# leducthanhig/image-restoration-models

Measured on AMD Instinct MI355X. Metric: images/sec + PSNR, Restormer motion-deblur 1280x720, higher is better.
Workload: dtype f32 (1x1 convs: fp32 emulated by 3 fp16 MFMAs on hi/lo operand splits with fp32 accumulation, error vs float64 at the level of an fp32 chain; everything else exact f32; value_exact_f32: f32 MFMA everywhere); 1 GPU; Restormer motion-deblur (WithBias LN, 26.13M params, synthetic weights seed 42) on 1280x720x3 uint8 GoPro-shaped synthetic frames; 6 tiles 512x512 (overlap 96) per frame; a step = 4 frame(s) per GPU, their 24 tiles in one batched forward; global_batch=4, tile=512, overlap=96, parallelism=per-image shard x1, no data-path collective

## Files before the change

### image-restoration-models_amd/_hip.py

```python
from __future__ import annotations

import ctypes as C
import os

import torch

_HERE = os.path.dirname(os.path.abspath(__file__))
LIB_PATH = os.path.join(_HERE, "libirm_hip.so")

ACT_NONE, ACT_RELU, ACT_GELU, ACT_SILU, ACT_RELU6 = 0, 1, 2, 3, 4
LN_NONE, LN_WITHBIAS, LN_BIASFREE = 0, 1, 2

_P, _L, _I, _F, _D = C.c_void_p, C.c_long, C.c_int, C.c_float, C.c_double

SIGNATURES = {
    "irm_version": [],
    "irm_ln_stats_f32": [_P, _L, _P, _I, _I, _I, _F, _P],
    "irm_gemm1x1_f32": [_P, _L, _P, _L, _P, _L, _P, _L, _P, _P, _P, _P, _I, _I, _I, _I, _I, _I, _I, _I, _P, _F, _P, _P],
    "irm_gemm1x1_f16x3_f32": [_P, _L, _P, _L, _P, _L, _P, _L, _P, _P, _P, _P, _I, _I, _I, _I, _I, _I, _I, _I, _P, _F, _P, _P],
    "irm_ln_split_f16": [_P, _L, _P, _P, _I, _F, _F, _P, _I, _I, _I, _P],
    "irm_ln_gemm_presplit_f16x3_f32": [_P, _P, _L, _P, _P, _I, _F, _F, _P, _L, _P, _F, _I, _I, _I, _I, _I, _P],
    "irm_ln_gemm_presplit_cl_f16x3_f32": [_P, _P, _L, _P, _P, _I, _F, _F, _P, _L, _P, _F, _I, _I, _I, _I, _I, _I, _P],
    "irm_gdfn_tail_f16x3_f32": [_P, _L, _P, _P, _P, _P, _L, _F, _I, _I, _I, _I, _I, _I, _P],
    "irm_gemm_presplit_f16x3_f32": [_P, _P, _P, _L, _P, _F, _I, _I, _I, _I, _I, _I, _I, _I, _P],
# ... 30 lines not shown
    "irm_selective_scan_f32": [_P, _P, _P, _P, _P, _P, _P, _P, _P, _P, _P, _I, _I, _I, _I, _I, _I, _P],
    "irm_losh_combine_f32": [_P, _P, _P, _P, _P, _P, _P, _P, _L, _P, _L, _I, _I, _I, _I, _F, _P],
    "irm_window_blend": [_P, _P, _P, _P, _I, _P, _P, _I, _I, _I, _I, _I, _I, _I, _I, _I, _I, _F, _F, _P],
    "irm_window_blend_scaled": [_P, _P, _P, _P, _I, _P, _P, _I, _I, _I, _I, _I, _I, _I, _I, _I, _I, _I, _F, _F, _P],
    "irm_frame_metrics": [_P, _P, _I, _I, _I, _I, _I, _D, _P, _P, _P, _L, _P],
    "irm_imresize_bicubic": [_P, _I, _P, _I, _P, _P, _P, _P, _I, _I, _I, _I, _I, _I, _P],
    "irm_frame_metrics_basicsr": [_P, _P, _I, _I, _I, _I, _I, _I, _I, _I, _P, _P, _P, _L, _P],
    "irm_niqe_features": [_P, _I, _I, _I, _I, _I, _I, _I, _P, _P, _P, _L, _P],
    "irm_dihedral_chop_f32": [_P, _P, _P, _L, _I, _I, _I, _I, _I, _I, _I, _P],
    "irm_ensemble_merge_f32": [_P, _P, _P, _L, _I, _I, _I, _I, _I, _I, _P],
}

SIGNATURES_HALF = {
    "irm_conv3x3_h_in_f32": [_P, _P, _L, _P, _L, _P, _I, _I, _I, _I, _I, _I, _P],
    "irm_conv3x3_h_f16": [_P, _F, _P, _L, _P, _L, _P, _L, _P, _I, _I, _I, _I, _I, _I, _I, _I, _P],
    "irm_conv3x3_h_out_f32": [_P, _P, _L, _P, _L, _P, _L, _P, _I, _I, _I, _I, _I, _I, _P],
}

SIGNATURES_FRAMES = {
    "irm_frame_minmax_f32": [_P, _L, _P, _P, _L, _P],
    "irm_tile_extract_f32": [_P, _P, _P, _P, _P, _I, _I, _I, _I, _I, _I, _I, _I, _I, _P],
    "irm_window_blend_f32": [_P, _P, _P, _P, _P, _I, _I, _I, _I, _I, _I, _I, _I, _I, _I, _I, _P],
}

SIGNATURES_GRAM = {
    "irm_dw_gram_cm_f16x3_f32": [_P, _L, _P, _P, _P, _P, _I, _I, _I, _I, _I, _P],
}

SIGNATURES_YUV = {
    "irm_yuv420_to_rgb_f32": [_P, _P, _P, _I, _L, _L, _I, _I, _I, _I, _I, _I, _I, _I, _P, _P],
    "irm_rgb_f32_to_yuv420": [_P, _P, _P, _P, _I, _L, _L, _I, _I, _I, _I, _I, _I, _I, _I, _P],
}

_lib = None


class HipLibraryError(RuntimeError):
    pass


def load():
    global _lib, LIB_PATH
    if _lib is None:
        if os.environ.get("IRM_HIP_LIB"):
            LIB_PATH = os.path.abspath(os.environ["IRM_HIP_LIB"])
        if not os.path.exists(LIB_PATH):
            raise HipLibraryError(
                f"{LIB_PATH} not found: build it with `python -c 'import __graft_entry__ as g; g.build()'` "
                "(make -C image-restoration-models_amd/csrc).  There is no CPU fallback.")
        lib = C.CDLL(LIB_PATH)
        for name, argtypes in {**SIGNATURES, **SIGNATURES_HALF, **SIGNATURES_FRAMES, **SIGNATURES_GRAM,
                               **SIGNATURES_YUV}.items():
            fn = getattr(lib, name)
            fn.argtypes = argtypes
            fn.restype = _I
        _lib = lib
    return _lib


def _stream() -> int:
    return torch.cuda.current_stream().cuda_stream


def ptr(t):
    if t is None:
        return None
    if isinstance(t, int):
        return t
    assert t.is_cuda, "HIP kernels need device tensors"
    return t.data_ptr()


def call(name: str, *args):
    rc = getattr(load(), name)(*args, _stream())
    if rc != 0:
        raise HipLibraryError(f"{name} failed with status {rc} "
                              f"({'invalid arguments' if rc == -1 else 'HIP launch error'})")



def pack_gemm_weight(w: torch.Tensor) -> torch.Tensor:
    w = w.detach().reshape(w.shape[0], -1).float()
    m, k = w.shape
    mt, ks = (m + 15) // 16, 4 * ((k + 15) // 16)
    wpad = torch.zeros(mt * 16, ks * 4, dtype=torch.float32, device=w.device)
# ... 402 lines not shown
```

### image-restoration-models_amd/csrc/conv3x3_f16.hip

```cpp
#include "conv_epilogue.h"


#define CF_TH 8
#define CF_TW IRM_CONV_TW
#define CF_PLANE 400
#define CF_HC 34
#define CF_NP 340
#define CF_PXB 160
#define CF_RAWB (7 * 512 * 16)
#define CF_IMGB (CF_NP * CF_PXB)
#define CF_NRAW 7


__device__ __forceinline__ float cf_res(float v, float r, int mode) {
    if (mode == 1) return v + r;
    if (mode == 2) return r - v;
    return fminf(fmaxf(tanhf(v) + r, -1.0f), 1.0f);
}

struct ConvF16Args {
    const float* Wp;
    const float* X; long x_bs;
    float* Y; long y_bs;
    const float* R; long r_bs;
    const float* bias;
    int Ci, Co, H, W, mtiles, S;
    int relu1, res_mode, relu2, store_mode, tiles_x;
    float inv_s;
    float slope;
    int ps_r;
};


template <int CT, int NCH = 1>
__global__ __launch_bounds__(512, 2) void conv3x3_f16x3_kernel(ConvF16Args a) {
    constexpr int TT = CT * NCH;
    constexpr int NG = 3 * NCH;
    constexpr int WGB = 3 * CT * 2048;
    constexpr int NW = (WGB / 16 + 511) / 512;
    extern __shared__ __attribute__((aligned(16))) float smem[];
    char* lds = reinterpret_cast<char*>(smem);
    char* raw = lds;
    char* img = lds + CF_RAWB;
    char* wbuf = img + CF_IMGB;

    const int tid = threadIdx.x, lane = tid & 63, wave = __builtin_amdgcn_readfirstlane(tid >> 6);
    const int g = lane >> 4, r = lane & 15;
    const int b = blockIdx.z;
    const int ty0 = (blockIdx.x / a.tiles_x) * CF_TH, tx0 = (blockIdx.x % a.tiles_x) * CF_TW;
    const float* X = a.X + (long)b * a.x_bs;
    const long plane = (long)a.H * a.W;
    const int S = a.S;
    const int nchunks = (a.mtiles + TT - 1) / TT;
    const int my_chunks = (nchunks - (int)blockIdx.y + (int)gridDim.y - 1) / (int)gridDim.y;

    long xoff[CF_NRAW];
    int xch[CF_NRAW];
    bool xok[CF_NRAW];
#pragma unroll
    for (int j = 0; j < CF_NRAW; ++j) {
        const int q = j * 512 + tid;
        const int ch = q / 100, rem = q - ch * 100, row = rem / 10, chunk = rem - row * 10;
        const int gy = ty0 - 1 + row, gx = tx0 - 4 + chunk * 4;
        xch[j] = ch;
        xok[j] = q < 3200 && gy >= 0 && gy < a.H && gx >= 0 && gx < a.W;
        xoff[j] = (long)ch * plane + (long)gy * a.W + gx;
    }
    const float* const zero_page = irm_zero_page;
    auto issue_raw = [&](int s) {
#pragma unroll
        for (int j = 0; j < CF_NRAW; ++j) {
            const bool ok = xok[j] && s * 32 + xch[j] < a.Ci;
            const float* src = ok ? X + (long)s * 32 * plane + xoff[j] : zero_page;
            __builtin_amdgcn_global_load_lds((const __attribute__((address_space(1))) void*)src,
                                             (__attribute__((address_space(3))) void*)(raw + (j * 512 + wave * 64) * 16), 16, 0, 0);
        }
    };
    auto issue_w = [&](int mt0, int n) {
        const int sc = n / 3, tg = n - 3 * sc, s = sc / NCH, chn = sc - s * NCH;
#pragma unroll
        for (int j = 0; j < NW; ++j) {
            const int cb = min(j * 512 + wave * 64, WGB / 16 - 64);
            const int q = cb + lane;
            const int ct = q / 384, rem = q - ct * 384;
            const int mt = min(mt0 + chn * CT + ct, a.mtiles - 1);
            const float* src = a.Wp + ((((long)mt * S + s) * 9 + tg * 3) * 2) * 256 + rem * 4;
            __builtin_amdgcn_global_load_lds((const __attribute__((address_space(1))) void*)src,
                                             (__attribute__((address_space(3))) void*)(wbuf + (n & 1) * WGB + cb * 16), 16, 0, 0);
        }
    };

    f32x4 acc[2][TT];
    float* Y = a.Y + (long)b * a.y_bs;
    const float* R = a.R ? a.R + (long)b * a.r_bs : nullptr;

    for (int ci = 0; ci < my_chunks; ++ci) {
        const int mt0 = ((int)blockIdx.y + ci * (int)gridDim.y) * TT;
#pragma unroll
        for (int p = 0; p < 2; ++p)
#pragma unroll
            for (int c = 0; c < TT; ++c) acc[p][c] = (f32x4){0.f, 0.f, 0.f, 0.f};
        __builtin_amdgcn_s_barrier();
        issue_raw(0);
        issue_w(mt0, 0);
        for (int s = 0; s < S; ++s) {
            irm_wait_vmcnt<0>();
            __builtin_amdgcn_s_barrier();
#pragma unroll
            for (int it = 0; it < 3; ++it) {
                const int item = it * 512 + tid;
                if (item < 4 * CF_NP) {
                    const int cg = item / CF_NP, px = item - cg * CF_NP;
                    const int row = px / CF_HC, col = px - row * CF_HC;
                    const float* rp = reinterpret_cast<const float*>(raw) + (8 * cg) * CF_PLANE + row * 40 + col + 3;
                    irm_h8 hi, lo;
                    float xs[8];
#pragma unroll
                    for (int e = 0; e < 8; ++e) xs[e] = irm_sat_h(__fmul_rn(rp[e * CF_PLANE], 0.0625f));
                    irm_split8(xs, hi, lo);
                    *reinterpret_cast<irm_h8*>(img + px * CF_PXB + cg * 16) = hi;
                    *reinterpret_cast<irm_h8*>(img + px * CF_PXB + 64 + cg * 16) = lo;
                }
            }
            asm volatile("s_waitcnt lgkmcnt(0)" ::: "memory");
            __builtin_amdgcn_s_barrier();
            issue_w(mt0, NG * s + 1);
            if (s + 1 < S) issue_raw(s + 1);
#pragma unroll
            for (int gi = 0; gi < NG; ++gi) {
                const int n = NG * s + gi, tg = gi % 3, chn = gi / 3;
                if (gi == 1) {
                    if (s + 1 < S) irm_wait_vmcnt<CF_NRAW>(); else irm_wait_vmcnt<0>();
                    __builtin_amdgcn_s_barrier();
                    issue_w(mt0, n + 1);
                } else if (gi > 1) {
                    irm_wait_vmcnt<0>();
                    __builtin_amdgcn_s_barrier();
                    if (gi + 1 < NG || s + 1 < S) issue_w(mt0, n + 1);
                }
                const char* wb = wbuf + (n & 1) * WGB;
#pragma unroll
                for (int tl = 0; tl < 3; ++tl) {
                    const int dy = tg, dx = tl;
                    irm_h8 ah[2], al[2];
#pragma unroll
                    for (int p = 0; p < 2; ++p) {
                        const int pi = (wave + dy) * CF_HC + 16 * p + r + dx;
                        ah[p] = *reinterpret_cast<const irm_h8*>(img + pi * CF_PXB + 16 * g);
                        al[p] = *reinterpret_cast<const irm_h8*>(img + pi * CF_PXB + 64 + 16 * g);
                    }
#pragma unroll
                    for (int c = 0; c < CT; ++c) {
                        const irm_h8 wh = *reinterpret_cast<const irm_h8*>(wb + ((c * 3 + tl) * 2) * 1024 + lane * 16);
                        const irm_h8 wl = *reinterpret_cast<const irm_h8*>(wb + ((c * 3 + tl) * 2 + 1) * 1024 + lane * 16);
#pragma unroll
                        for (int p = 0; p < 2; ++p) {
                            f32x4& t = acc[p][chn * CT + c];
                            t = irm_mfma3_f16(ah[p], al[p], wh, wl, t);
                        }
                    }
                }
            }
        }
#pragma unroll
        for (int c = 0; c < TT; ++c) {
            const int co = (mt0 + c) * 16 + r;
            const bool row_ok = mt0 + c < a.mtiles && co < a.Co;
            const float bv = (a.bias && row_ok) ? a.bias[co] : 0.0f;
#pragma unroll
            for (int p = 0; p < 2; ++p) {
                const int y = ty0 + wave, x = tx0 + p * 16 + g * 4;
                float v[4];
#pragma unroll
                for (int e = 0; e < 4; ++e) {
                    v[e] = fmaf(acc[p][c][e], a.inv_s, bv);
                    if (a.relu1 == 1) v[e] = fmaxf(v[e], 0.0f);
                    else if (a.relu1 == 2) v[e] = v[e] > 0.0f ? v[e] : v[e] * a.slope;
                }
                if (!row_ok || y >= a.H || x >= a.W) continue;
                if (a.store_mode == 0) {
                    const long off = (long)co * plane + (long)y * a.W + x;
                    if (a.res_mode) {
                        const float4 rr = *reinterpret_cast<const float4*>(R + off);
                        const float rv[4] = {rr.x, rr.y, rr.z, rr.w};
#pragma unroll
                        for (int e = 0; e < 4; ++e) v[e] = cf_res(v[e], rv[e], a.res_mode);
                    }
                    if (a.relu2) {
#pragma unroll
                        for (int e = 0; e < 4; ++e) v[e] = fmaxf(v[e], 0.0f);
                    }
                    *reinterpret_cast<float4*>(Y + off) = make_float4(v[0], v[1], v[2], v[3]);
                } else if (a.store_mode == 1) {
                    const int oh = a.H >> 1, ow = a.W >> 1;
                    const long op = (long)oh * ow;
                    const int oc = co * 4 + (y & 1) * 2;
                    const long o = (long)(y >> 1) * ow + (x >> 1);
                    *reinterpret_cast<float2*>(Y + (long)oc * op + o) = make_float2(v[0], v[2]);
                    *reinterpret_cast<float2*>(Y + (long)(oc + 1) * op + o) = make_float2(v[1], v[3]);
                } else if (a.ps_r == 2) {
                    const int ow = a.W * 2;
                    const long op = (long)a.H * 2 * ow;
                    const int oc = co >> 2, i = (co >> 1) & 1, jx = co & 1;
                    float* o = Y + (long)oc * op + (long)(2 * y + i) * ow + 2 * x + jx;
#pragma unroll
                    for (int e = 0; e < 4; ++e) o[2 * e] = v[e];
                } else {
                    const int pr = a.ps_r, ow = a.W * pr;
                    const long op = (long)a.H * pr * ow;
                    const int oc = co / (pr * pr), i = (co / pr) % pr, jx = co % pr;
                    float* o = Y + (long)oc * op + (long)(pr * y + i) * ow + pr * x + jx;
#pragma unroll
                    for (int e = 0; e < 4; ++e) o[pr * e] = v[e];
                }
            }
        }
    }
}

template <int CT, int NCH = 1>
static int launch_conv_f16(const ConvF16Args& a, int B, int ygroups, hipStream_t stream) {
    const size_t lds = (size_t)CF_RAWB + CF_IMGB + 2 * (3 * CT * 2048);
    static_assert((size_t)CF_RAWB + CF_IMGB + 2 * (3 * CT * 2048) <= 160 * 1024, "LDS");
    IRM_ALLOW_BIG_LDS((&conv3x3_f16x3_kernel<CT, NCH>));
    const int tiles_y = (a.H + CF_TH - 1) / CF_TH;
    dim3 grid(a.tiles_x * tiles_y, ygroups, B);
    hipLaunchKernelGGL((conv3x3_f16x3_kernel<CT, NCH>), grid, dim3(512), lds, stream, a);
    return irm_launch_status();
}

extern "C" int irm_conv3x3_f16x3_ep_f32(const float* wp_split, float inv_scale, const float* x, long x_bs, float* y,
                                        long y_bs, const float* res, long r_bs, const float* bias, int B, int Ci, int Co,
                                        int H, int W, int act1, float slope, int res_mode, int relu2, int store_mode,
                                        int shuffle, int ct, int ygroups, hipStream_t stream) {
    ConvF16Args a;
    if (int rc = irm_conv_common(a, wp_split, x, x_bs, y, y_bs, res, r_bs, bias, B, Ci, Co, H, W, act1, slope, res_mode,
                                 relu2, store_mode, shuffle, ct, ygroups)) return rc;
    if ((W & 3) || (x_bs & 3) || (y_bs & 3) || (r_bs & 3)) return IRM_EINVAL;
    if (!irm_aligned16(x) || !irm_aligned16(y) || !irm_aligned16(res) || !irm_aligned16(wp_split)) return IRM_EINVAL;
    a.S = (Ci + 31) / 32; a.inv_s = inv_scale;
    switch (ct) {
        case 1: return launch_conv_f16<1>(a, B, ygroups, stream);
        case 2: return launch_conv_f16<2>(a, B, ygroups, stream);
        case 3: return launch_conv_f16<3>(a, B, ygroups, stream);
        case 4: return launch_conv_f16<4>(a, B, ygroups, stream);
        case 8: return launch_conv_f16<4, 2>(a, B, ygroups, stream);
        case 12: return launch_conv_f16<4, 3>(a, B, ygroups, stream);
        default: return IRM_EINVAL;
    }
}

extern "C" int irm_conv3x3_f16x3_f32(const float* wp_split, float inv_scale, const float* x, long x_bs, float* y, long y_bs,
                                     const float* res, long r_bs, const float* bias, int B, int Ci, int Co, int H, int W,
                                     int relu1, int res_mode, int relu2, int store_mode, int ct, int ygroups,
                                     hipStream_t stream) {
    return irm_conv3x3_f16x3_ep_f32(wp_split, inv_scale, x, x_bs, y, y_bs, res, r_bs, bias, B, Ci, Co, H, W, relu1 ? 1 : 0,
                                    0.0f, res_mode, relu2, store_mode, 2, ct, ygroups, stream);
}
```

### image-restoration-models_amd/ops.py

```python
from __future__ import annotations

import os

import torch

from . import _hip
from ._hip import ACT_GELU, ACT_NONE, ACT_RELU, ACT_RELU6, ACT_SILU, LN_BIASFREE, LN_NONE, LN_WITHBIAS


class KernelTimer:

    def __init__(self, detail=False, only=None):
        self.records = []
        self.detail = detail
        self.only = None if only is None else frozenset(only)
        self._chain = {}
        self._done = {}
        self._since = 0

    def _fold(self, k, e0, e1, fl, by):
        d = self._done.setdefault(k, dict(launches=0, ms=0.0, flops=0.0, bytes=0.0))
        d["launches"] += 1
        d["ms"] += e0.elapsed_time(e1)
        d["flops"] += fl
# ... 400 lines not shown
        ygroups = max(1, min(nchunks, -(-target_blocks() // blocks)))
    return ct, ygroups


def conv3x3(wp, x, y, ci: int, co: int, *, bias=None, relu1=False, res=None, res_mode=0, relu2=False,
            store_mode=0, ct: int | None = None, ygroups: int | None = None, leaky: float | None = None, shuffle: int = 2):
    _chk(x, "x"), _chk(y, "y")
    B, _, H, W = x.shape
    nbytes = 4.0 * B * H * W * (ci + co + (co if res is not None else 0))
    if leaky is not None and relu1:
        raise ValueError("conv3x3: relu1 and leaky are exclusive")
    act1, slope = (2, float(leaky)) if leaky is not None else (int(bool(relu1)), 0.0)
    extra = (f" ps{shuffle}" if shuffle != 2 else "") + (f" leaky{slope:g}" if leaky is not None else "")
    if isinstance(wp, _hip.ConvWeight):
        aligned = (W % 4 == 0 and _bs(x) % 4 == 0 and _bs(y) % 4 == 0 and _bs(res) % 4 == 0 and x.data_ptr() % 16 == 0
                   and y.data_ptr() % 16 == 0 and (res is None or res.data_ptr() % 16 == 0))
        if wp.raw is not None and aligned and store_mode == 0 and act1 < 2:
            _launch("conv3x3_thin", 18.0 * B * ci * co * H * W, nbytes, "irm_conv3x3_thin_f32", _hip.ptr(wp.raw), _hip.ptr(x),
                    _bs(x), _hip.ptr(y), _bs(y), _hip.ptr(res), _bs(res), _hip.ptr(bias), B, ci, co, H, W, int(relu1),
                    int(res_mode), int(relu2), tag=f"ci{ci} co{co} {H}x{W} B{B}")
            return
        wp = (wp.split, wp.inv_scale) if (wp.split is not None and aligned) else wp.exact
    if isinstance(wp, tuple):
        kernel, entry, lead = "conv3x3_f16x3", "irm_conv3x3_f16x3_ep_f32", (_hip.ptr(wp[0]), float(wp[1]))
    else:
        kernel, entry, lead = "conv3x3", "irm_conv3x3_ep_f32", (_hip.ptr(wp),)
    ct, ygroups = plan_conv3x3(co, H, W, B, split=isinstance(wp, tuple), ct=ct, ygroups=ygroups)
    _launch(kernel, 18.0 * B * ci * co * H * W, nbytes, entry, *lead, _hip.ptr(x), _bs(x), _hip.ptr(y), _bs(y),
            _hip.ptr(res), _bs(res), _hip.ptr(bias), B, ci, co, H, W, act1, slope, int(res_mode), int(relu2),
            int(store_mode), int(shuffle), ct, ygroups,
            tag=f"ci{ci} co{co} {H}x{W} B{B} ct{ct} yg{ygroups} st{store_mode}{extra}")


def transpose(src: torch.Tensor, dst: torch.Tensor, R: int, C: int):
    B = src.shape[0]
    _launch("transpose", 0.0, 8.0 * B * R * C, "irm_transpose_f32", _hip.ptr(src), src.stride(0), _hip.ptr(dst),
            dst.stride(0), B, R, C, tag=f"R{R} C{C} B{B}")


def scan_is_flat(D: int, N: int, R: int) -> bool:
    return (N, R) in ((1, 4), (16, 4)) and D % 64 != 0


def scan_plan(B: int, L: int, D: int, flat: bool = False):
    DB = (D + 63) // 64
    waves = -(-4 * D // 64) if flat else 4 * DB
    nchunk = max(1, min(-(-L // 32), -(-3072 // (B * waves))))
    chunk = max(32, -(-(-(-L // nchunk)) // 8) * 8)
    return chunk, -(-L // chunk), DB


def selective_scan(xT, pT, ids, dtw, dtb, A, Dskip, yT, state, sdt, ysum, B, L, D, N, R, chunk):
    flops = B * 4.0 * L * D * (2 * R + 9 * N + 12)
    nbytes = 4.0 * B * L * (D + 4 * (R + 2 * N) + 4 * D)
    _launch("selective_scan", flops, nbytes, "irm_selective_scan_f32", _hip.ptr(xT), _hip.ptr(pT), _hip.ptr(ids),
            _hip.ptr(dtw), _hip.ptr(dtb), _hip.ptr(A), _hip.ptr(Dskip), _hip.ptr(yT), _hip.ptr(state), _hip.ptr(sdt),
            _hip.ptr(ysum), B, L, D, N, R, chunk, tag=f"L{L} D{D} N{N} B{B} chunk{chunk}")


def losh_combine(ysum, gw, gb, gate, yT, nw, nb, z, out, B, L, D, nchunk, eps=1e-5):
    _chk(z, "z"), _chk(out, "out")
    _launch("losh_combine", 12.0 * B * L * D, 4.0 * B * L * D * 6, "irm_losh_combine_f32", _hip.ptr(ysum), _hip.ptr(gw),
            _hip.ptr(gb), _hip.ptr(gate), _hip.ptr(yT), _hip.ptr(nw), _hip.ptr(nb), _hip.ptr(z), _bs(z), _hip.ptr(out),
            _bs(out), B, L, D, nchunk, float(eps), tag=f"L{L} D{D} B{B}")


# ... 58 lines not shown
```

### image-restoration-models_amd/restormer/restormer.py

```python
from __future__ import annotations

import os

import torch
import torch.nn as nn

from .. import _hip, ops, unet
from ..host import ModelHost, f32

SYNTH_RULES = (
    (r"^output\.weight$", "gain", 0.02),
    (r"^skip_conv\.weight$", "gain", 0.5),
)


def _hidden(dim, factor):
    return int(dim * factor)


class _Norm(nn.Module):

    def __init__(self, dim, kind):
        super().__init__()
        self.body = nn.Module()
# ... 117 lines not shown
    SYNTH_RULES = SYNTH_RULES

    def __init__(self, inp_channels=3, out_channels=3, dim=48, num_blocks=(4, 6, 6, 8),
                 num_refinement_blocks=4, heads=(1, 2, 4, 8), ffn_expansion_factor=2.66, bias=False,
                 LayerNorm_type="WithBias", dual_pixel_task=False):
        super().__init__()
        f, ln = ffn_expansion_factor, LayerNorm_type
        d1, d2, d3, d4 = dim, dim * 2, dim * 4, dim * 8
        self.inp_channels, self.out_channels, self.dim = inp_channels, out_channels, dim
        self.patch_embed = _Proj(inp_channels, d1, bias=False)
        self.encoder_level1 = _stage(d1, heads[0], num_blocks[0], f, bias, ln)
        self.down1_2 = _Resample(d1, d1 // 2)
        self.encoder_level2 = _stage(d2, heads[1], num_blocks[1], f, bias, ln)
        self.down2_3 = _Resample(d2, d2 // 2)
        self.encoder_level3 = _stage(d3, heads[2], num_blocks[2], f, bias, ln)
        self.down3_4 = _Resample(d3, d3 // 2)
        self.latent = _stage(d4, heads[3], num_blocks[3], f, bias, ln)
        self.up4_3 = _Resample(d4, d4 * 2)
        self.reduce_chan_level3 = nn.Conv2d(d4, d3, 1, bias=bias)
        self.decoder_level3 = _stage(d3, heads[2], num_blocks[2], f, bias, ln)
        self.up3_2 = _Resample(d3, d3 * 2)
        self.reduce_chan_level2 = nn.Conv2d(d3, d2, 1, bias=bias)
        self.decoder_level2 = _stage(d2, heads[1], num_blocks[1], f, bias, ln)
        self.up2_1 = _Resample(d2, d2 * 2)
        self.decoder_level1 = _stage(d2, heads[0], num_blocks[0], f, bias, ln)
        self.refinement = _stage(d2, heads[0], num_refinement_blocks, f, bias, ln)
        self.dual_pixel_task = dual_pixel_task
        if dual_pixel_task:
            self.skip_conv = nn.Conv2d(d1, d2, 1, bias=bias)
        self.output = nn.Conv2d(d2, out_channels, 3, padding=1, bias=bias)
        self._split = False
        self.max_tiles_per_batch = 12
        self.hip_graph = True
        self._tap = None

    def _build(self):
        self._split = not os.environ.get("IRM_GEMM_EXACT")
        pk = {name: pack_block(m, self._split) for name, m in self.named_modules() if isinstance(m, TransformerBlock)}
        pk.update(unet.pack_unet(self))
        for name in ("reduce_chan_level3", "reduce_chan_level2"):
            if self._split and _hip.split_is_safe(getattr(self, name).weight):
                pk[name + "_s"] = _hip.pack_gemm_weight_split(getattr(self, name).weight)
        return pk

    def _block(self, blk: TransformerBlock, w: dict, x: torch.Tensor, have_stats: bool = False,
               want_stats: bool = True) -> bool:
        B, C, H, W = x.shape
        N = H * W
        dev = x.device
        heads = blk.attn.num_heads
        hid = blk.ffn.hidden
        fuse = ops.can_fuse_stats(C)
        stats = self._buf("stats", B * 2 * N, dev)
        big_a = self._buf("scratch_a", B * max(3 * C, 2 * hid) * N, dev)
        big_b = self._buf("scratch_b", B * max(3 * C, hid) * N, dev)
        qkv = big_a[:B * 3 * C * N].view(B, 3 * C, H, W)
        qkv2 = big_b[:B * 3 * C * N].view(B, 3 * C, H, W)
        split = self._split and N % 4 == 0
        s_qkv, s_pin, s_pout = split and "qkv_s" in w, split and "pin_s" in w, split and "pout_s" in w
        s_fold = split and w.get("mfold_split", False)
        presplit = split and "qkv_ps" in w and ops.can_presplit(C, N)
        if presplit:
            xs = self._buf("xsplit", B * C * N, dev)
            frag, out_scale, s_x = w["qkv_ps"]
            ops.ln_gemm_presplit(frag, x, qkv, 3 * C, C, w["n1w"], w["n1b"], blk.norm1.mode, s_x, out_scale=out_scale,
                                 bias=w["qkv_b"], xs=xs)
# ... 64 lines not shown
        heads, hid = blk.attn.num_heads, blk.ffn.hidden
        qkv = self._buf("scratch_a", B * 3 * C * N, dev).view(B, 3 * C, H, W)
        tm = ops.can_qk_tile_major(C, heads, H, W)
        fa = "gdfn_fa" in w
        assert not (x_tm or y_tm) or (tm and fa), "tile-major x / y: only between the kernels that understand them"
        v_tm = tm and fa
        gram_in_qkv = tm and "gram_s" in w and ops.can_qkv_gram(C, heads, H, W)
        _, nchunk, rec = ops.mdta_plan(B, C, heads, N)
        nready = None
        if gram_in_qkv:
            nchunk = (H // 8) * (W // 32) // ops.QKV_GRAM_NCH
        part = self._buf("gram_part", B * heads * nchunk * rec, dev)
        if gram_in_qkv:
            nready = ops.qkv_gram_cm(w["qkv_f"], x, qkv, w["gram_s"], part, C, ln_mode=blk.norm1.mode, x_tm=x_tm, v_tm=v_tm)
        else:
            ops.qkv_dw_fused(w["qkv_f"], x, qkv, C, 3 * C, ln_mode=blk.norm1.mode, tm=tm, x_tm=x_tm, v_tm=v_tm)
        gsum = self._buf("gram_sum", B * heads * rec, dev)
        mfold_n = ops.mfold_numel(C)
        mfold = self._zeros(("mfold", C, B), B * mfold_n, dev)
        s_fold = w.get("mfold_split", False)
        if fa:
            mfrag = self._zeros(("mfold_frag", C, B), B * ops.mfold_frag_numel(C), dev)
            ops.mdta_fold(qkv, part, gsum, w["temp"], w["wout"], mfrag, C, heads, gram_scale=w.get("gram_s"), frag=True, tm=tm,
                          nchunk_ready=nready)
            ops.attn_gdfn_fused(w["gdfn_fa"], x, qkv[:, 2 * C:], mfrag, alt, C, hid, ln_mode=blk.norm2.mode,
                                bias_o=w["wout_b"], bias=w["pout_b"], x_tm=x_tm, v_tm=v_tm, y_tm=y_tm)
            return alt
        ops.mdta_fold(qkv, part, gsum, w["temp"], w["wout"], mfold, C, heads, split=s_fold, gram_scale=w.get("gram_s"), tm=tm,
                      nchunk_ready=nready)
        ops.gemm1x1(mfold, qkv[:, 2 * C:], x, C, C, res=x, bias=w["wout_b"], w_bs=mfold_n, split=s_fold)
        ops.gdfn_fused(w["gdfn_f"], x, alt, C, hid, ln_mode=blk.norm2.mode, bias=w["pout_b"])
        return alt

    def _run_stage(self, name, pk, x, have_stats=False):
        names = (name,) if isinstance(name, str) else tuple(name)
        blocks = [(f"{n}.{i}", blk) for n in names for i, blk in enumerate(getattr(self, n))]
        B, C, H, W = x.shape
        if (len(blocks) and all("gdfn_f" in pk[k] for k, _ in blocks) and ops.can_fuse_gdfn(C, W) and (H * W) % 4 == 0
                and len({blk.attn.num_heads for _, blk in blocks}) == 1):
            cur, alt = x, self._buf(f"alt_{C}", B * C * H * W, x.device).view(B, C, H, W)
            heads = blocks[0][1].attn.num_heads
            act_tm = all("gdfn_fa" in pk[k] for k, _ in blocks) and ops.can_qk_tile_major(C, heads, H, W)
            for i, (k, blk) in enumerate(blocks):
                out = self._block_fused(blk, pk[k], cur, alt, x_tm=act_tm and i > 0, y_tm=act_tm and i + 1 < len(blocks))
                cur, alt = out, cur
            if cur is not x:
                x.copy_(cur)
                if ops.TIMER is not None:
                    ops.TIMER.break_chain()
            return False
        for n in names:
            stage = getattr(self, n)
            for i, blk in enumerate(stage):
                have_stats = self._block(blk, pk[f"{n}.{i}"], x, have_stats, want_stats=i + 1 < len(stage))
        return have_stats

    @torch.no_grad()
    def forward(self, inp_img: torch.Tensor) -> torch.Tensor:
        self._require_cuda(inp_img)
        x = inp_img.float().contiguous()
        if x.shape[2] % 8 or x.shape[3] % 8:
            raise ValueError("Restormer needs H and W to be multiples of 8 (the tiler pads, utils.pad)")
        pk = self._pack()
        tap = self.__dict__.get("_tap")
        return unet.forward(self, x, pk, lambda names, t, level: self._run_stage(names, pk, t),
                            None if tap is None else lambda t: tap.__setitem__("refinement", t.clone()))
```

### image-restoration-models_amd/unet.py

```python
from __future__ import annotations

import torch

from . import _hip, ops
from .host import f32

RESAMPLE = ("down1_2", "down2_3", "down3_4", "up4_3", "up3_2", "up2_1")


def pack_unet(model) -> dict:
    pk = {name: _hip.pack_conv3x3(getattr(model, name).body[0].weight) for name in RESAMPLE}
    pk["patch_embed"] = _hip.pack_conv3x3(model.patch_embed.proj.weight)
    pk["output"] = _hip.pack_conv3x3(model.output.weight)
    pk["output_b"] = f32(model.output.bias)
    for name in ("reduce_chan_level3", "reduce_chan_level2") + (("skip_conv",) if model.dual_pixel_task else ()):
        pk[name] = _hip.pack_gemm_weight(getattr(model, name).weight)
        pk[name + "_b"] = f32(getattr(model, name).bias)
    return pk


def _reduce_chan(pk, name, cat, dec, c):
    split = name + "_s" in pk and (cat.shape[2] * cat.shape[3]) % 4 == 0
    ops.gemm1x1(pk[name + "_s" if split else name], cat, dec, c, 2 * c, bias=pk[name + "_b"], split=split)


def forward(model, x, pk, run_stage, after_trunk=None):
    B, Cin, H, W = x.shape
    dev = x.device
    d1, d2, d3, d4 = model.dim, model.dim * 2, model.dim * 4, model.dim * 8
    H2, W2, H3, W3, H4, W4 = H // 2, W // 2, H // 4, W // 4, H // 8, W // 8

    def buf(name, ch, h, w):
        return model._buf(name, B * ch * h * w, dev).view(B, ch, h, w)

    cat1 = buf("cat1", 2 * d1, H, W)
    cat2 = buf("cat2", 2 * d2, H2, W2)
    cat3 = buf("cat3", 2 * d3, H3, W3)
    lat = buf("latent", d4, H4, W4)
    dec3 = buf("dec3", d3, H3, W3)
    dec2 = buf("dec2", d2, H2, W2)

    e1 = cat1[:, d1:]
    ops.conv3x3(pk["patch_embed"], x, e1, Cin, d1)
    if model.dual_pixel_task:
        e1_in = buf("enc1_in", d1, H, W)
        e1_in.copy_(e1)
        if ops.TIMER is not None:
            ops.TIMER.break_chain()
    run_stage(("encoder_level1",), e1, 0)
    e2 = cat2[:, d2:]
    ops.conv3x3(pk["down1_2"], e1, e2, d1, d1 // 2, store_mode=1)
    run_stage(("encoder_level2",), e2, 1)
    e3 = cat3[:, d3:]
    ops.conv3x3(pk["down2_3"], e2, e3, d2, d2 // 2, store_mode=1)
    run_stage(("encoder_level3",), e3, 2)
    ops.conv3x3(pk["down3_4"], e3, lat, d3, d3 // 2, store_mode=1)
    run_stage(("latent",), lat, 3)

    ops.conv3x3(pk["up4_3"], lat, cat3[:, :d3], d4, d4 * 2, store_mode=2)
    _reduce_chan(pk, "reduce_chan_level3", cat3, dec3, d3)
    run_stage(("decoder_level3",), dec3, 2)
    ops.conv3x3(pk["up3_2"], dec3, cat2[:, :d2], d3, d3 * 2, store_mode=2)
    _reduce_chan(pk, "reduce_chan_level2", cat2, dec2, d2)
    run_stage(("decoder_level2",), dec2, 1)
    ops.conv3x3(pk["up2_1"], dec2, cat1[:, :d1], d2, d2 * 2, store_mode=2)
    run_stage(("decoder_level1", "refinement"), cat1, 0)
    if after_trunk is not None:
        after_trunk(cat1)

    out = torch.empty(B, model.out_channels, H, W, dtype=torch.float32, device=dev)
    if model.dual_pixel_task:
        ops.gemm1x1(pk["skip_conv"], e1_in, cat1, d2, d1, res=cat1, bias=pk["skip_conv_b"])
        ops.conv3x3(pk["output"], cat1, out, d2, model.out_channels, bias=pk["output_b"])
    else:
        ops.conv3x3(pk["output"], cat1, out, d2, model.out_channels, bias=pk["output_b"], res=x, res_mode=1)
    return out
```

### include/irm_hip.h

```cpp
#ifndef IRM_HIP_H
#define IRM_HIP_H

#ifdef __cplusplus
extern "C" {
#endif

typedef struct ihipStream_t* irm_stream_t;

#define IRM_OK 0
#define IRM_EINVAL (-1)
#define IRM_ELAUNCH (-2)

#define IRM_ACT_NONE 0
#define IRM_ACT_RELU 1
#define IRM_ACT_GELU 2
#define IRM_ACT_SILU 3

#define IRM_LN_NONE 0
#define IRM_LN_WITHBIAS 1
#define IRM_LN_BIASFREE 2

int irm_version(void);

int irm_ln_stats_f32(const float* x, long x_bs, float* stats, int B, int C, int N, float eps,
// ... 128 lines not shown
                          const float* res, long r_bs, float* y, long y_bs, int B, int C, int N, int act,
                          irm_stream_t stream);
int irm_conv3x3_s2_f32(const float* x, long x_bs, const float* w, float* y, long y_bs, int B, int Ci, int Co, int H,
                       int W, irm_stream_t stream);
int irm_dwconv3x3_s2_f32(const float* x, long x_bs, const float* w, float* y, long y_bs, int B, int C, int H, int W,
                         irm_stream_t stream);
int irm_upsample_add_f32(const float* src, long s_bs, const float* add, long a_bs, float* out, long o_bs, int B, int C,
                         int Hs, int Ws, int scale, irm_stream_t stream);

int irm_dihedral_chop_f32(const float* src, const int* table, float* dst, long dst_pixels, int B, int C, int H, int W,
                          int P, int max_ph, int max_pw, irm_stream_t stream);
int irm_ensemble_merge_f32(const float* pred, const int* table, float* out, long pred_pixels, int B, int Co, int H,
                           int W, int P, int scale, irm_stream_t stream);

int irm_transpose_f32(const float* in, long in_bs, float* out, long out_bs, int B, int R, int C,
                      irm_stream_t stream);

int irm_selective_scan_f32(const float* xT, const float* pT, const int* ids, const float* dtw, const float* dtb,
                           const float* A, const float* Dskip, float* yT, float* state, float* sdt, float* ysum,
                           int B, int L, int D, int N, int R, int chunk, irm_stream_t stream);

int irm_losh_combine_f32(float* ysum, const float* gw, const float* gb, float* gate, const float* yT,
                         const float* nw, const float* nb, const float* z, long z_bs, float* out, long out_bs,
                         int B, int L, int D, int nchunk, float eps, irm_stream_t stream);

#include "irm_hip_half.h"

#include "irm_hip_frames.h"

#include "irm_hip_gram.h"

#include "irm_hip_yuv.h"

#ifdef __cplusplus
}
#endif
#endif
```

Baseline: 22.45 images/s.

## Emit tile-major stage inputs directly from down/up-sample 3x3 convs

Adds a channels-last/tile-major variant of the split-fp16 3x3 conv that writes its pixel-unshuffle/shuffle output straight into the tile-major layout the fused transformer stages consume. While loading input it can also write a tile-major copy of the encoder-level1 activations into the cat1 skip buffer. This lets encoder_level2 and decoder_level1+refinement start in tile-major form and skip their first layout conversion. The cost is scattered strided stores and extra side writes in the conv epilogue, plus more buffers.

```diff
diff --git a/image-restoration-models_amd/_hip.py b/image-restoration-models_amd/_hip.py
--- a/image-restoration-models_amd/_hip.py
+++ b/image-restoration-models_amd/_hip.py
@@ -86,6 +86,10 @@
     "irm_rgb_f32_to_yuv420": [_P, _P, _P, _P, _I, _L, _L, _I, _I, _I, _I, _I, _I, _I, _I, _P],
 }
 
+SIGNATURES_STAGE = {
+    "irm_conv3x3_f16x3_cl_f32": [_P, _F, _P, _L, _P, _L, _I, _I, _P, _L, _I, _I, _P, _I, _I, _I, _I, _I, _I, _F, _I, _I, _I, _P],
+}
+
 _lib = None
 
 
@@ -104,7 +108,7 @@
                 "(make -C image-restoration-models_amd/csrc).  There is no CPU fallback.")
         lib = C.CDLL(LIB_PATH)
         for name, argtypes in {**SIGNATURES, **SIGNATURES_HALF, **SIGNATURES_FRAMES, **SIGNATURES_GRAM,
-                               **SIGNATURES_YUV}.items():
+                               **SIGNATURES_YUV, **SIGNATURES_STAGE}.items():
             fn = getattr(lib, name)
             fn.argtypes = argtypes
             fn.restype = _I
diff --git a/image-restoration-models_amd/csrc/conv3x3_f16.hip b/image-restoration-models_amd/csrc/conv3x3_f16.hip
--- a/image-restoration-models_amd/csrc/conv3x3_f16.hip
+++ b/image-restoration-models_amd/csrc/conv3x3_f16.hip
@@ -32,8 +32,14 @@
 };
 
 
-template <int CT, int NCH = 1>
-__global__ __launch_bounds__(512, 2) void conv3x3_f16x3_kernel(ConvF16Args a) {
+struct ConvF16Cl {
+    int Cb, c_off;
+    float* xcl; long xcl_bs;
+    int Cb_x, c_off_x;
+};
+
+template <int CT, int NCH, bool CL>
+__device__ __forceinline__ void conv3x3_f16x3_body(const ConvF16Args& a, const ConvF16Cl& cl) {
     constexpr int TT = CT * NCH;
     constexpr int NG = 3 * NCH;
     constexpr int WGB = 3 * CT * 2048;
@@ -94,7 +100,10 @@
     float* Y = a.Y + (long)b * a.y_bs;
     const float* R = a.R ? a.R + (long)b * a.r_bs : nullptr;
 
+    float* const xside = (CL && cl.xcl) ? cl.xcl + (long)b * cl.xcl_bs + (long)blockIdx.x * (CF_TH * CF_TW) * cl.Cb_x + cl.c_off_x
+                                        : nullptr;
     for (int ci = 0; ci < my_chunks; ++ci) {
+        const bool side = CL && xside && blockIdx.y == 0 && ci == 0;
         const int mt0 = ((int)blockIdx.y + ci * (int)gridDim.y) * TT;
 #pragma unroll
         for (int p = 0; p < 2; ++p)
@@ -117,6 +126,23 @@
                     float xs[8];
 #pragma unroll
                     for (int e = 0; e < 8; ++e) xs[e] = irm_sat_h(__fmul_rn(rp[e * CF_PLANE], 0.0625f));
+                    if (CL && side && row >= 1 && row <= CF_TH && col >= 1 && col <= CF_TW) {
+                        const int ch = s * 32 + 8 * cg;
+                        float xr[8];
+#pragma unroll
+                        for (int e = 0; e < 8; ++e) xr[e] = rp[e * CF_PLANE];
+                        float* o = xside + ((long)(row - 1) * CF_TW + (col - 1)) * cl.Cb_x + ch;
+#pragma unroll
+                        for (int h = 0; h < 2; ++h) {
+                            if (ch + 4 * h + 4 <= a.Ci) {
+                                *reinterpret_cast<float4*>(o + 4 * h) = make_float4(xr[4 * h], xr[4 * h + 1], xr[4 * h + 2], xr[4 * h + 3]);
+                            } else {
+#pragma unroll
+                                for (int e = 0; e < 4; ++e)
+                                    if (ch + 4 * h + e < a.Ci) o[4 * h + e] = xr[4 * h + e];
+                            }
+                        }
+                    }
                     irm_split8(xs, hi, lo);
                     *reinterpret_cast<irm_h8*>(img + px * CF_PXB + cg * 16) = hi;
                     *reinterpret_cast<irm_h8*>(img + px * CF_PXB + 64 + cg * 16) = lo;
@@ -178,6 +204,22 @@
                     else if (a.relu1 == 2) v[e] = v[e] > 0.0f ? v[e] : v[e] * a.slope;
                 }
                 if (!row_ok || y >= a.H || x >= a.W) continue;
+                if (CL) {
+                    if (a.store_mode == 1) {
+                        const int ow = a.W >> 1, oy = y >> 1, ox = x >> 1;
+                        const int oc = co * 4 + (y & 1) * 2;
+                        float* o = Y + (((long)(oy >> 3) * (ow >> 5) + (ox >> 5)) * 256 + (oy & 7) * 32 + (ox & 31)) * cl.Cb + cl.c_off + oc;
+                        *reinterpret_cast<float2*>(o) = make_float2(v[0], v[1]);
+                        *reinterpret_cast<float2*>(o + cl.Cb) = make_float2(v[2], v[3]);
+                    } else {
+                        const int ow = a.W * 2;
+                        const int oc = co >> 2, oy = 2 * y + ((co >> 1) & 1), ox = 2 * x + (co & 1);
+                        float* o = Y + (((long)(oy >> 3) * (ow >> 5) + (ox >> 5)) * 256 + (oy & 7) * 32 + (ox & 31)) * cl.Cb + cl.c_off + oc;
+#pragma unroll
+                        for (int e = 0; e < 4; ++e) o[(long)2 * e * cl.Cb] = v[e];
+                    }
+                    continue;
+                }
                 if (a.store_mode == 0) {
                     const long off = (long)co * plane + (long)y * a.W + x;
                     if (a.res_mode) {
@@ -216,6 +258,16 @@
             }
         }
     }
+}
+
+template <int CT, int NCH = 1>
+__global__ __launch_bounds__(512, 2) void conv3x3_f16x3_kernel(ConvF16Args a) {
+    conv3x3_f16x3_body<CT, NCH, false>(a, ConvF16Cl{});
+}
+
+template <int CT, int NCH = 1>
+__global__ __launch_bounds__(512, 2) void conv3x3_f16x3_cl_kernel(ConvF16Args a, ConvF16Cl cl) {
+    conv3x3_f16x3_body<CT, NCH, true>(a, cl);
 }
 
 template <int CT, int NCH = 1>
@@ -257,3 +309,45 @@
     return irm_conv3x3_f16x3_ep_f32(wp_split, inv_scale, x, x_bs, y, y_bs, res, r_bs, bias, B, Ci, Co, H, W, relu1 ? 1 : 0,
                                     0.0f, res_mode, relu2, store_mode, 2, ct, ygroups, stream);
 }
+
+template <int CT, int NCH = 1>
+static int launch_conv_f16_cl(const ConvF16Args& a, const ConvF16Cl& cl, int B, int ygroups, hipStream_t stream) {
+    const size_t lds = (size_t)CF_RAWB + CF_IMGB + 2 * (3 * CT * 2048);
+    IRM_ALLOW_BIG_LDS((&conv3x3_f16x3_cl_kernel<CT, NCH>));
+    const int tiles_y = (a.H + CF_TH - 1) / CF_TH;
+    dim3 grid(a.tiles_x * tiles_y, ygroups, B);
+    hipLaunchKernelGGL((conv3x3_f16x3_cl_kernel<CT, NCH>), grid, dim3(512), lds, stream, a, cl);
+    return irm_launch_status();
+}
+
+extern "C" int irm_conv3x3_f16x3_cl_f32(const float* wp_split, float inv_scale, const float* x, long x_bs, float* y,
+                                        long y_bs, int Cb, int c_off, float* xcl, long xcl_bs, int Cb_x, int c_off_x,
+                                        const float* bias, int B, int Ci, int Co, int H, int W, int act1, float slope,
+                                        int store_mode, int ct, int ygroups, hipStream_t stream) {
+    ConvF16Args a;
+    if (store_mode != 1 && store_mode != 2) return IRM_EINVAL;
+    if (int rc = irm_conv_common(a, wp_split, x, x_bs, y, y_bs, nullptr, 0, bias, B, Ci, Co, H, W, act1, slope, 0, 0,
+                                 store_mode, 2, ct, ygroups)) return rc;
+    if ((W & 3) || (x_bs & 3) || (y_bs & 3) || x_bs < (long)Ci * H * W) return IRM_EINVAL;
+    if (!irm_aligned16(x) || !irm_aligned16(y) || !irm_aligned16(wp_split)) return IRM_EINVAL;
+    const long oh = store_mode == 1 ? H / 2 : 2L * H, ow = store_mode == 1 ? W / 2 : 2L * W;
+    const int oc = store_mode == 1 ? 4 * Co : Co / 4;
+    if ((oh % CF_TH) || (ow % CF_TW)) return IRM_EINVAL;
+    if (Cb <= 0 || (Cb & 3) || c_off < 0 || (c_off & 3) || (long)c_off + oc > Cb || y_bs < oh * ow * Cb) return IRM_EINVAL;
+    if (xcl) {
+        if ((H % CF_TH) || (W % CF_TW) || !irm_aligned16(xcl)) return IRM_EINVAL;
+        if (Cb_x <= 0 || (Cb_x & 3) || c_off_x < 0 || (c_off_x & 7) || (long)c_off_x + Ci > Cb_x) return IRM_EINVAL;
+        if ((xcl_bs & 3) || xcl_bs < (long)H * W * Cb_x) return IRM_EINVAL;
+    }
+    a.S = (Ci + 31) / 32; a.inv_s = inv_scale;
+    const ConvF16Cl cl{Cb, c_off, xcl, xcl_bs, Cb_x, c_off_x};
+    switch (ct) {
+        case 1: return launch_conv_f16_cl<1>(a, cl, B, ygroups, stream);
+        case 2: return launch_conv_f16_cl<2>(a, cl, B, ygroups, stream);
+        case 3: return launch_conv_f16_cl<3>(a, cl, B, ygroups, stream);
+        case 4: return launch_conv_f16_cl<4>(a, cl, B, ygroups, stream);
+        case 8: return launch_conv_f16_cl<4, 2>(a, cl, B, ygroups, stream);
+        case 12: return launch_conv_f16_cl<4, 3>(a, cl, B, ygroups, stream);
+        default: return IRM_EINVAL;
+    }
+}
diff --git a/image-restoration-models_amd/ops.py b/image-restoration-models_amd/ops.py
--- a/image-restoration-models_amd/ops.py
+++ b/image-restoration-models_amd/ops.py
@@ -456,6 +456,38 @@
             tag=f"ci{ci} co{co} {H}x{W} B{B} ct{ct} yg{ygroups} st{store_mode}{extra}")
 
 
+def _dense16(t) -> bool:
+    return t.data_ptr() % 16 == 0 and t.stride(0) % 4 == 0
+
+
+def can_conv3x3_cl(wp, x, store_mode: int) -> bool:
+    _, _, H, W = x.shape
+    oh, ow = (H // 2, W // 2) if store_mode == 1 else (2 * H, 2 * W)
+    return (isinstance(wp, _hip.ConvWeight) and wp.raw is None and wp.split is not None and store_mode in (1, 2)
+            and H % 2 == 0 and W % 4 == 0 and oh % 8 == 0 and ow % 32 == 0 and _dense16(x))
+
+
+def conv3x3_cl(wp, x, y, ci: int, co: int, *, store_mode: int, c_off: int = 0, xcl=None, c_off_x: int = 0, bias=None,
+               ct: int | None = None, ygroups: int | None = None):
+    _chk(x, "x"), _chk(y, "y")
+    B, _, H, W = x.shape
+    oh, ow = (H // 2, W // 2) if store_mode == 1 else (2 * H, 2 * W)
+    oc = 4 * co if store_mode == 1 else co // 4
+    assert can_conv3x3_cl(wp, x, store_mode) and y.shape[0] == B and y.shape[2:] == (oh, ow) and _dense16(y)
+    assert c_off % 4 == 0 and c_off + oc <= y.shape[1] and y.shape[1] % 4 == 0
+    nbytes = 4.0 * B * H * W * (ci + co)
+    if xcl is not None:
+        _chk(xcl, "xcl")
+        assert xcl.shape[0] == B and xcl.shape[2:] == (H, W) and H % 8 == 0 and W % 32 == 0 and _dense16(xcl)
+        assert c_off_x % 8 == 0 and c_off_x + ci <= xcl.shape[1] and xcl.shape[1] % 4 == 0
+        nbytes += 4.0 * B * H * W * ci
+    ct, ygroups = plan_conv3x3(co, H, W, B, split=True, ct=ct, ygroups=ygroups)
+    _launch("conv3x3_f16x3", 18.0 * B * ci * co * H * W, nbytes, "irm_conv3x3_f16x3_cl_f32", _hip.ptr(wp.split),
+            float(wp.inv_scale), _hip.ptr(x), _bs(x), _hip.ptr(y), _bs(y), y.shape[1], int(c_off), _hip.ptr(xcl), _bs(xcl),
+            0 if xcl is None else xcl.shape[1], int(c_off_x), _hip.ptr(bias), B, ci, co, H, W, 0, 0.0, int(store_mode), ct,
+            ygroups, tag=f"ci{ci} co{co} {H}x{W} B{B} ct{ct} yg{ygroups} st{store_mode} cl" + ("+x" if xcl is not None else ""))
+
+
 def transpose(src: torch.Tensor, dst: torch.Tensor, R: int, C: int):
     B = src.shape[0]
     _launch("transpose", 0.0, 8.0 * B * R * C, "irm_transpose_f32", _hip.ptr(src), src.stride(0), _hip.ptr(dst),
diff --git a/image-restoration-models_amd/restormer/restormer.py b/image-restoration-models_amd/restormer/restormer.py
--- a/image-restoration-models_amd/restormer/restormer.py
+++ b/image-restoration-models_amd/restormer/restormer.py
@@ -173,6 +173,7 @@
         self._split = False
         self.max_tiles_per_batch = 12
         self.hip_graph = True
+        self.stage_tm = True
         self._tap = None
 
     def _build(self):
@@ -303,18 +304,33 @@
         ops.gdfn_fused(w["gdfn_f"], x, alt, C, hid, ln_mode=blk.norm2.mode, bias=w["pout_b"])
         return alt
 
-    def _run_stage(self, name, pk, x, have_stats=False):
+    def _stage_blocks(self, name):
         names = (name,) if isinstance(name, str) else tuple(name)
-        blocks = [(f"{n}.{i}", blk) for n in names for i, blk in enumerate(getattr(self, n))]
+        return names, [(f"{n}.{i}", blk) for n in names for i, blk in enumerate(getattr(self, n))]
+
+    def _stage_plan(self, blocks, pk, C, H, W):
+        fused = (len(blocks) > 0 and all("gdfn_f" in pk[k] for k, _ in blocks) and ops.can_fuse_gdfn(C, W) and (H * W) % 4 == 0
+                 and len({blk.attn.num_heads for _, blk in blocks}) == 1)
+        act_tm = (fused and all("gdfn_fa" in pk[k] for k, _ in blocks)
+                  and ops.can_qk_tile_major(C, blocks[0][1].attn.num_heads, H, W))
+        return fused, act_tm
+
+    def _stage_takes_tm(self, name, pk, B, C, H, W) -> bool:
+        return bool(self.stage_tm) and self._stage_plan(self._stage_blocks(name)[1], pk, C, H, W)[1]
+
+    def _run_stage(self, name, pk, x, have_stats=False, x_tm=None):
+        names, blocks = self._stage_blocks(name)
         B, C, H, W = x.shape
-        if (len(blocks) and all("gdfn_f" in pk[k] for k, _ in blocks) and ops.can_fuse_gdfn(C, W) and (H * W) % 4 == 0
-                and len({blk.attn.num_heads for _, blk in blocks}) == 1):
+        fused, act_tm = self._stage_plan(blocks, pk, C, H, W)
+        assert x_tm is None or (act_tm and x_tm.shape == x.shape), "a tile-major stage input needs a stage that reads it"
+        if fused:
             cur, alt = x, self._buf(f"alt_{C}", B * C * H * W, x.device).view(B, C, H, W)
-            heads = blocks[0][1].attn.num_heads
-            act_tm = all("gdfn_fa" in pk[k] for k, _ in blocks) and ops.can_qk_tile_major(C, heads, H, W)
+            if x_tm is not None:
+                cur = x_tm
             for i, (k, blk) in enumerate(blocks):
-                out = self._block_fused(blk, pk[k], cur, alt, x_tm=act_tm and i > 0, y_tm=act_tm and i + 1 < len(blocks))
-                cur, alt = out, cur
+                out = self._block_fused(blk, pk[k], cur, alt, x_tm=act_tm and (i > 0 or x_tm is not None),
+                                        y_tm=act_tm and i + 1 < len(blocks))
+                cur, alt = out, (x if cur is x_tm else cur)
             if cur is not x:
                 x.copy_(cur)
                 if ops.TIMER is not None:
@@ -334,5 +350,5 @@
             raise ValueError("Restormer needs H and W to be multiples of 8 (the tiler pads, utils.pad)")
         pk = self._pack()
         tap = self.__dict__.get("_tap")
-        return unet.forward(self, x, pk, lambda names, t, level: self._run_stage(names, pk, t),
+        return unet.forward(self, x, pk, lambda names, t, level, x_tm=None: self._run_stage(names, pk, t, x_tm=x_tm),
                             None if tap is None else lambda t: tap.__setitem__("refinement", t.clone()))
diff --git a/image-restoration-models_amd/unet.py b/image-restoration-models_amd/unet.py
--- a/image-restoration-models_amd/unet.py
+++ b/image-restoration-models_amd/unet.py
@@ -40,7 +40,15 @@
     dec3 = buf("dec3", d3, H3, W3)
     dec2 = buf("dec2", d2, H2, W2)
 
+    takes_tm = None if model.dual_pixel_task else getattr(model, "_stage_takes_tm", None)
+
+    def tm(names, ch, h, w):
+        return takes_tm is not None and takes_tm(names, pk, B, ch, h, w)
+
     e1 = cat1[:, d1:]
+    tm_e2 = tm(("encoder_level2",), d2, H2, W2) and ops.can_conv3x3_cl(pk["down1_2"], e1, 1)
+    tm_cat1 = (tm_e2 and tm(("decoder_level1", "refinement"), 2 * d1, H, W) and H % 8 == 0 and W % 32 == 0
+               and ops.can_conv3x3_cl(pk["up2_1"], dec2, 2))
     ops.conv3x3(pk["patch_embed"], x, e1, Cin, d1)
     if model.dual_pixel_task:
         e1_in = buf("enc1_in", d1, H, W)
@@ -49,8 +57,14 @@
             ops.TIMER.break_chain()
     run_stage(("encoder_level1",), e1, 0)
     e2 = cat2[:, d2:]
-    ops.conv3x3(pk["down1_2"], e1, e2, d1, d1 // 2, store_mode=1)
-    run_stage(("encoder_level2",), e2, 1)
+    if tm_e2:
+        e2_tm = buf("e2_tm", d2, H2, W2)
+        cat1_tm = buf("cat1_tm", 2 * d1, H, W) if tm_cat1 else None
+        ops.conv3x3_cl(pk["down1_2"], e1, e2_tm, d1, d1 // 2, store_mode=1, xcl=cat1_tm, c_off_x=d1)
+        run_stage(("encoder_level2",), e2, 1, x_tm=e2_tm)
+    else:
+        ops.conv3x3(pk["down1_2"], e1, e2, d1, d1 // 2, store_mode=1)
+        run_stage(("encoder_level2",), e2, 1)
     e3 = cat3[:, d3:]
     ops.conv3x3(pk["down2_3"], e2, e3, d2, d2 // 2, store_mode=1)
     run_stage(("encoder_level3",), e3, 2)
@@ -63,8 +77,12 @@
     ops.conv3x3(pk["up3_2"], dec3, cat2[:, :d2], d3, d3 * 2, store_mode=2)
     _reduce_chan(pk, "reduce_chan_level2", cat2, dec2, d2)
     run_stage(("decoder_level2",), dec2, 1)
-    ops.conv3x3(pk["up2_1"], dec2, cat1[:, :d1], d2, d2 * 2, store_mode=2)
-    run_stage(("decoder_level1", "refinement"), cat1, 0)
+    if tm_cat1:
+        ops.conv3x3_cl(pk["up2_1"], dec2, cat1_tm, d2, d2 * 2, store_mode=2, c_off=0)
+        run_stage(("decoder_level1", "refinement"), cat1, 0, x_tm=cat1_tm)
+    else:
+        ops.conv3x3(pk["up2_1"], dec2, cat1[:, :d1], d2, d2 * 2, store_mode=2)
+        run_stage(("decoder_level1", "refinement"), cat1, 0)
     if after_trunk is not None:
         after_trunk(cat1)
 
diff --git a/include/irm_hip.h b/include/irm_hip.h
--- a/include/irm_hip.h
+++ b/include/irm_hip.h
@@ -184,6 +184,8 @@
 
 #include "irm_hip_yuv.h"
 
+#include "irm_hip_stage.h"
+
 #ifdef __cplusplus
 }
 #endif
diff --git a/include/irm_hip_stage.h b/include/irm_hip_stage.h
--- /dev/null
+++ b/include/irm_hip_stage.h
@@ -0,0 +1,6 @@
+#pragma once
+
+int irm_conv3x3_f16x3_cl_f32(const float* wp_split, float inv_scale, const float* x, long x_bs, float* y, long y_bs, int Cb,
+                             int c_off, float* xcl, long xcl_bs, int Cb_x, int c_off_x, const float* bias, int B, int Ci,
+                             int Co, int H, int W, int act1, float slope, int store_mode, int ct, int ygroups,
+                             irm_stream_t stream);
```

Measured after the change: 22.42 images/s. No clear change (-0.1%).
